# EdoardoBotta/RQ-VAE-Recommender

Hardware: AMD Instinct MI355X
Metric: item-embeddings quantized/sec (RQ-VAE fwd+bwd) (higher is better)
Workload: dtype f32 (MLP GEMMs f16x2-emulated)

## Files before the change

include/rqhip.h:

```cpp
#ifndef RQHIP_H
#define RQHIP_H

#include <stddef.h>
#include <stdint.h>

#ifdef __cplusplus
extern "C" {
#endif

#define RQHIP_VERSION 462

#define RQHIP_OK 0
#define RQHIP_EARG (-1)
#define RQHIP_EUNSUPPORTED (-2)
#define RQHIP_EWORKSPACE (-3)

#define RQHIP_MODE_EVAL 0
#define RQHIP_MODE_STE 1
#define RQHIP_MODE_ROTATION 2
#define RQHIP_MODE_GUMBEL 3

typedef void *rqhip_stream_t;

int rqhip_version(void);
// ... 336 lines not shown
    float *loss_rows;
    void *workspace;
    size_t workspace_bytes;
    const unsigned *a_row_max;
    int a_row_parts;
    unsigned *c_row_max;
    unsigned *c_col_max;
} rqhip_gemm_args;
int rqhip_gemm_split_supported(int Nc, int R);
size_t rqhip_weight_image_bytes(int Nc, int R, int arith);
int rqhip_weight_images(const rqhip_image_job *jobs, int n_jobs, rqhip_stream_t stream);
int rqhip_maxima(const float *A, const float *Y, float *masked_out, int64_t M, int R, unsigned *row_max, unsigned *col_max,
                 rqhip_stream_t stream);
size_t rqhip_gemm_split_recon_workspace_bytes(int64_t M, int Nc);
int rqhip_gemm_split_ex(const rqhip_gemm_args *args, rqhip_stream_t stream);
size_t rqhip_weight_planes_bytes(int Nc, int R);
int rqhip_weight_planes(const float *w, int rows, int cols, int transpose, void *planes, size_t planes_bytes,
                        rqhip_stream_t stream);
int rqhip_gemm_split(const float *A, int64_t M, int R, const void *planes, int Nc, int relu, float *C,
                     rqhip_stream_t stream);
int rqhip_gemm_split_recon(const float *A, int64_t M, int R, const void *planes, int Nc, const float *X, float row_scale,
                           float *G, float *loss_rows, void *workspace, size_t workspace_bytes, rqhip_stream_t stream);
int rqhip_recon_rescale_rows(const float *g_out, int64_t B, int N, float row_scale, float *g_spec, rqhip_stream_t stream);
int rqhip_recon_rescale_rows_ex(const float *g_out, int64_t B, int N, float row_scale, float *g_spec, unsigned *row_max,
                                int row_parts, unsigned *col_max, rqhip_stream_t stream);

typedef struct {
    int64_t B;
    int D;
    int H;
// ... 63 lines not shown
```

rq-vae-recommender_amd/csrc/gemm_split.hip:

```cpp
#include "rqhip_common.h"

namespace rqhip {

typedef float gs_f32x16 __attribute__((ext_vector_type(16)));
typedef float gs_f32x4 __attribute__((ext_vector_type(4)));
typedef float gs_f32x2 __attribute__((ext_vector_type(2)));
typedef __bf16 gs_bf16x8 __attribute__((ext_vector_type(8)));
typedef __bf16 gs_bf16x2 __attribute__((ext_vector_type(2)));
typedef _Float16 gs_f16x8 __attribute__((ext_vector_type(8)));
typedef _Float16 gs_f16x2 __attribute__((ext_vector_type(2)));
typedef unsigned gs_u32x2 __attribute__((ext_vector_type(2)));
typedef unsigned gs_u32x4 __attribute__((ext_vector_type(4)));
typedef int gs_i32x4 __attribute__((ext_vector_type(4)));

constexpr int kGsUB = 2;
constexpr int kGsK = 16;
constexpr int kGsColmaxLds = 1024;
constexpr int kGsTailWords = kWeightImageTailWords;

__device__ __forceinline__ void gs_split2(float a, float b, unsigned &h, unsigned &m, unsigned &l) {
    const gs_bf16x2 hh = __builtin_convertvector(gs_f32x2{a, b}, gs_bf16x2);
    h = __builtin_bit_cast(unsigned, hh);
    const float ra = a - __builtin_bit_cast(float, h << 16), rb = b - __builtin_bit_cast(float, h & 0xffff0000u);
    const gs_bf16x2 mm = __builtin_convertvector(gs_f32x2{ra, rb}, gs_bf16x2);
// ... 179 lines not shown
    int R, Nc;
    int n_col_tiles;
    unsigned n_big, n_tiles;
    int rt_big;
    unsigned *counter;
    int n_queues;
    int rt_fastest;
    int static_tiles;
    const float *X;
    float *rowsum;
    float row_scale;
    const unsigned *a_max;
    int a_parts;
    const int *b_exp;
    unsigned *c_rowmax, *c_colmax;
};

#ifndef GS_PROBE
#define GS_PROBE 0
#endif
#ifndef GS_PROLOGUE_ORDER
#define GS_PROLOGUE_ORDER 1
#endif
#ifndef GS_FAST_EPILOGUE
#define GS_FAST_EPILOGUE 1
#endif
#ifndef GS_REGION_PAD
#define GS_REGION_PAD 32
#endif

__device__ __forceinline__ unsigned gs_row16_umax(unsigned v) {
// ... 689 lines not shown
        if (!(tile & kSmallBit)) {
            const int ct = p.rt_fastest ? (int)(tile / rt_big) : (int)(tile % nct), rt = p.rt_fastest ? (int)(tile % rt_big) : (int)(tile / nct);
            gs_tile2<EPI, kBigRows / 32, COLS>(p, sbuf, s_aexp, s_colmax, (long long)rt * kBigRows, ct * COLS);
        } else {
            const unsigned st = tile & ~kSmallBit;
            const int ct = p.rt_fastest ? (int)(st / rt_small) : (int)(st % nct), rt = p.rt_fastest ? (int)(st % rt_small) : (int)(st / nct);
            gs_tile2<EPI, kSmallRows / 32, COLS>(p, sbuf, s_aexp, s_colmax, (long long)p.rt_big * kBigRows + (long long)rt * kSmallRows, ct * COLS);
        }
    }
    if (lds_colmax) {
        for (int c = tid; c < p.Nc; c += kThreads)
            if (s_colmax[c]) atomicMax(p.c_colmax + c, s_colmax[c]);
    }
}

__global__ __launch_bounds__(256) void recon_rows_finish_kernel(const float *__restrict__ rowsum, int nct, long long M,
                                                                float *__restrict__ out) {
    const long long m = (long long)blockIdx.x * 256 + threadIdx.x;
    if (m >= M) return;
    float s = rowsum[m];
    for (int c = 1; c < nct; ++c) s = s + rowsum[(size_t)c * M + m];
    out[m] = s;
}

}

using namespace rqhip;

static int gs_cols(int Nc) { return Nc % 256 == 0 ? 256 : 128; }
static int gs_np(int arith) { return arith == RQHIP_SPLIT_F16X2 ? 2 : arith == RQHIP_SPLIT_BF16X3 ? 3 : 0; }
// ... 49 lines not shown
    if (M < 0 || R <= 0 || (R % 4) != 0 || R > 16384 || (M > 0 && !A) || (masked_out && !Y) || !al16(A) || !al16(Y) || !al16(masked_out)) {
        set_error("maxima: bad arguments (R = %d must be a multiple of 4, at most 16384; 16-byte aligned rows; masked_out needs Y)", R);
        return RQHIP_EARG;
    }
    if (M == 0 || (!row_max && !col_max && !masked_out)) return RQHIP_OK;
    long long blocks = (M + 3) / 4;
    const long long cap = (long long)cu_count() * 8;
    if (blocks > cap) blocks = cap;
    hipStream_t s = reinterpret_cast<hipStream_t>(stream);
    profile_begin(s, RQHIP_PROF_MAXIMA, 0.0, (double)M * R * 4 * ((Y ? 2 : 1) + (masked_out ? 1 : 0)));
    hipLaunchKernelGGL(maxima_kernel, dim3((unsigned)blocks), dim3(256), col_max ? (size_t)R * 4 : 0, s, A, Y, masked_out, (long long)M, R,
                       row_max, col_max);
    profile_end(s);
    RQ_CHECK_LAUNCH("maxima_kernel");
    return RQHIP_OK;
}

extern "C" size_t rqhip_gemm_split_recon_workspace_bytes(int64_t M, int Nc) {
    return (M > 0 && Nc > 0 && Nc % 256 == 0) ? (size_t)(Nc / 256) * (size_t)M * sizeof(float) : 0;
}

extern "C" int rqhip_gemm_split_ex(const rqhip_gemm_args *a, rqhip_stream_t stream) {
    if (!a) {
        set_error("gemm_split: null argument block");
        return RQHIP_EARG;
    }
    const int np = gs_np(a->arith), epi = a->epilogue;
    const int64_t M = a->M;
    const int R = a->R, Nc = a->Nc;
    if (!np || M < 0 || !a->image || (M > 0 && (!a->A || !a->C)) || !rqhip_gemm_split_supported(Nc, R) || epi < 0 || epi > 3) {
// ... 61 lines not shown
        rt_big = 0;
        tiny = a->tile_rows == -11;
        small_rows = tiny ? 32 : 64;
    }
    if (!tile2 && (a->tile_rows == 256 || a->tile_rows == 128)) rt_big = rt_all;
    if (!tile2 && (a->tile_rows == 64 || a->tile_rows == 32)) rt_big = 0;
    const long long rem_rows = M - rt_big * big_rows > 0 ? M - rt_big * big_rows : 0;
    const long long rt_small = (rem_rows + small_rows - 1) / small_rows;
    p.rt_big = (int)rt_big;
    p.n_big = (unsigned)(rt_big * p.n_col_tiles);
    p.n_tiles = p.n_big + (unsigned)(rt_small * p.n_col_tiles);
    size_t lds = (tile2 && !occ4) ? (size_t)2 * 4 * (128 * 4 + 32) * 4 : (size_t)2 * (np * 2 * (big_rows + cols) * 16);
    const size_t lds_epi = gs_epilogue_lds(waves, big_rows, wide ? 8 : cols / 64);
    if (lds < lds_epi) lds = lds_epi;
    const long long tiles = (long long)p.n_tiles;
    const int grid = (int)(tiles < slots ? tiles : slots);
    auto go = [&](auto kern) -> int {
        static LdsGrant grant;
        RQ_RETURN_IF_HIP(grant.ensure(reinterpret_cast<const void *>(kern), (int)lds));
        profile_begin(s, RQHIP_PROF_GEMM_SPLIT, 2.0 * (double)M * Nc * R, 4.0 * (double)M * (R + Nc * (epi >= 2 ? 2 : 1)));
        hipLaunchKernelGGL(kern, dim3(grid), dim3(64 * waves), lds, s, p);
        profile_end(s);
        RQ_CHECK_LAUNCH("gemm_split_kernel");
        return 0;
    };
    int rc;
    if (occ4) {
        rc = epi == 3 ? go(gemm_split_kernel<3, 256, 2, 8, 128>) : epi == 1 ? go(gemm_split_kernel<1, 256, 2, 8, 128>) : go(gemm_split_kernel<0, 256, 2, 8, 128>);
    } else if (wide) {
        rc = epi == 3 ? go(gemm_f16_kernel<3, 512>) : epi == 1 ? go(gemm_f16_kernel<1, 512>) : go(gemm_f16_kernel<0, 512>);
    } else if (tile2 && tiny) {
        rc = epi == 3 ? go(gemm_f16_kernel<3, 256, 1>) : epi == 2 ? go(gemm_f16_kernel<2, 256, 1>) : epi == 1 ? go(gemm_f16_kernel<1, 256, 1>)
                                                                                                          : go(gemm_f16_kernel<0, 256, 1>);
    } else if (tile2) {
        rc = epi == 3 ? go(gemm_f16_kernel<3>) : epi == 2 ? go(gemm_f16_kernel<2>) : epi == 1 ? go(gemm_f16_kernel<1>) : go(gemm_f16_kernel<0>);
    } else if (np == 2) {
        rc = epi == 3 ? go(gemm_split_kernel<3, 128, 2, 4>) : epi == 1 ? go(gemm_split_kernel<1, 128, 2, 4>) : go(gemm_split_kernel<0, 128, 2, 4>);
    } else {
        if (epi == 3) {
            set_error("gemm_split: the masked epilogue exists for RQHIP_SPLIT_F16X2 only");
            return RQHIP_EUNSUPPORTED;
        }
// ... 33 lines not shown
```

rq-vae-recommender_amd/modules/encoder.py:

```python
from typing import List

import torch
from torch import Tensor, nn

from modules.normalize import L2NormalizationLayer
from rqhip import linear as _lin
from rqhip import ops, torch_ops
from rqhip.linear import use_split_gemms


def _grad_sink(w: Tensor):
    from rqhip.dist import claim_grad_sink
    return claim_grad_sink(w)


def _adopt(gw: Tensor, sink) -> Tensor:
    return gw.view_as(gw) if sink is not None else gw


def _plain(layers) -> bool:
    return all((isinstance(l, nn.Linear) and l.bias is None) or isinstance(l, nn.ReLU) for l in layers)


class _LinearReLU(torch.autograd.Function):
# ... 4 lines not shown
        ctx.save_for_backward(x, w, y if zero_bias is not None else None)
        return y

    @staticmethod
    def backward(ctx, gy: Tensor):
        x, w, y = ctx.saved_tensors
        need_x, need_w = ctx.needs_input_grad[0], ctx.needs_input_grad[1]
        sink = _grad_sink(w) if need_w else None
        gx, gw = _lin.backward(gy, y, x, w, need_x, need_w, sink)
        return gx, (_adopt(gw, sink) if need_w else None), None


class _MLPStack(torch.autograd.Function):

    @staticmethod
    def forward(ctx, x: Tensor, target, relus, zero_bias, given, defer, *weights):
        from rqhip import _lib
        from rqhip import autograd as _ag
        assert _lin.dense_f32(x), "_MLPStack takes a contiguous, 16-byte aligned fp32 ROCm matrix (MLP._run re-homes what is not)"
        n, M, R = len(weights), x.shape[0], _lin.Route
        need_w = [bool(f) for f in ctx.needs_input_grad[6:]]
        need_in = [bool(ctx.needs_input_grad[0]) or any(need_w[:i]) for i in range(n)]
        stack_jobs = _lin.wgrad_jobs_ok(M, [tuple(w.shape) for i, w in enumerate(weights) if need_w[i]])
        plans = [_lin.plan_layer(M, w.shape[0], w.shape[1], relu=relus[i], operands_aligned=True, weight_ok=_lin.dense_f32(w),
                                 need_dgrad=need_in[i], need_wgrad=need_w[i], stack_jobs=stack_jobs) for i, w in enumerate(weights)]
        imgs = iter(_lin.images([(w, False) for w, p in zip(weights, plans) if p.fwd == R.SPLIT]
                                + [(w, True) for w, p in zip(weights, plans) if p.dgrad == R.SPLIT]))
        img_f = [next(imgs) if p.fwd == R.SPLIT else None for p in plans]
        img_t = [next(imgs) if p.dgrad == R.SPLIT else None for p in plans]
        emit = [p.fwd in (R.SPLIT, R.SEAM_OUT) and (plans[i + 1].wgrad_f16 if i + 1 < n else (target is not None and p.wgrad_f16))
                for i, p in enumerate(plans)]
        col_outs = _lin.col_slices([w.shape[0] if e else 0 for w, e in zip(weights, emit)], x.device)
        acts, scs = [x], [given if given is not None else _lin.Scales()]
        if _lin.f16() and (plans[0].fwd == R.SPLIT or plans[0].wgrad_f16):
            _lin.ensure_scales(x, scs[0], plans[0].fwd == R.SPLIT, plans[0].wgrad_f16)
        out = g_recon = g_scales = None
# ... 10 lines not shown
                y, ysc = _lin.chain_forward(a, w, relus[i], want_rows=want_rows, col_out=col_outs[i])
            elif p.fwd == R.SPLIT:
                y, _, ysc = _lin.gemm(a, img_f[i], w.shape[0], epilogue=_lib.EPI_RELU if relus[i] else _lib.EPI_STORE,
                                      a_scales=sc, want_rows=want_rows, col_out=col_outs[i])
            elif p.fwd == R.SMALL:
                y, ysc = _lin.small_forward(a, w, relus[i]), _lin.Scales()
            else:
                y, ysc = _lin.library_forward(a, w, relus[i], zero_bias(w.shape[0], a) if relus[i] else None), _lin.Scales()
            acts.append(y)
            scs.append(ysc)
            out = y
        ctx.has_target = target is not None
        ctx.save_for_backward(x, *weights, target if ctx.has_target else out)
        ctx.acts_mid, ctx.scs, ctx.relus = (acts[1:] if ctx.has_target else acts[1:-1]), scs, tuple(relus)
        ctx.plans, ctx.stack_jobs, ctx.img_t, ctx.need_in, ctx.need_w = plans, stack_jobs, img_t, need_in, need_w
        ctx.defer = bool(defer)
        ctx.g_recon, ctx.g_scales, ctx.consumed = g_recon, g_scales, False
        return out

    @staticmethod
    def backward(ctx, g_out: Tensor):
        from rqhip import _lib
        x, weights, tail = ctx.saved_tensors[0], ctx.saved_tensors[1:-1], ctx.saved_tensors[-1]
        n, R = len(weights), _lin.Route
        target = tail if ctx.has_target else None
        acts = [x] + list(ctx.acts_mid) + ([] if ctx.has_target else [tail])
        scs, relus, need_in, need_w, plans = ctx.scs, ctx.relus, ctx.need_in, ctx.need_w, ctx.plans
        g_out = g_out.contiguous()
        handed = _lin.take_grad_handoff(g_out) if target is None else None
        if g_out.data_ptr() % 16 != 0:
            g_out = g_out.clone()
        if handed is not None:
            g, gsc = g_out, handed
        elif target is None:
            g, gsc = g_out, _lin.Scales()
        elif not ctx.consumed:
            ctx.consumed = True
            gsc = ctx.g_scales
            g = ops.recon_rescale_rows(ctx.g_recon, g_out, ctx.row_scale, gsc.rows, gsc.cols)
        else:
            g = ops.recon_loss_backward(acts[-1].mm(weights[-1].t()), target, g_out, True, False)[0]
            gsc = _lin.Scales()
        emit = [i > 0 and p.dgrad in (R.SPLIT, R.SEAM_OUT) and plans[i - 1].wgrad_f16 for i, p in enumerate(plans)]
        col_outs = _lin.col_slices([w.shape[1] if e else 0 for w, e in zip(weights, emit)], g.device)
        premasked = (not relus[n - 1]) or handed is not None
        gws = [None] * n
        own = []
        for i in range(n - 1, -1, -1):
            w, a, p = weights[i], acts[i], plans[i]
            y = acts[i + 1] if (relus[i] and not premasked) else None
            mask_on_load = p.dgrad == R.SEAM_IN and y is not None
            g_unmasked = g
            if p.wgrad == R.JOBS and ctx.stack_jobs:
                if y is not None:
                    g, gsc = torch.ops.aten.threshold_backward(g, y, 0.0), _lin.Scales()
                own.append((i, _lin.WgradJob(w, g, a, None, None, _grad_sink(w))))
            elif p.wgrad == R.F16_SPLIT_BATCHED and y is None:
                gsc = _lin.ensure_scales(g, gsc, False, True)
                own.append((i, _lin.WgradJob(w, g, a, gsc.cols, _lin.ensure_scales(a, scs[i], False, True).cols, _grad_sink(w))))
            elif need_w[i]:
# ... 5 lines not shown
                g, gsc = torch.ops.aten.threshold_backward(g, y, 0.0), _lin.Scales()
            if not need_in[i]:
                g = None
                break
            lower_relu = i > 0 and relus[i - 1]
            lower_split = i > 0 and plans[i - 1].dgrad == R.SPLIT
            if p.dgrad in (R.SEAM_IN, R.SEAM_OUT):
                if p.dgrad == R.SEAM_IN:
                    src, msk = (g_unmasked, y) if (mask_on_load and (g is None or g is g_unmasked)) else (g, None)
                    g, gsc = _lin.chain_input_grad(src, w, g_mask=msk)
                    premasked = not lower_relu
                else:
                    g, gsc = _lin.chain_input_grad(g, w, out_mask=a if lower_relu else None, want_rows=lower_split, col_out=col_outs[i])
                    premasked = True
            elif p.dgrad == R.SPLIT:
                fuse = _lin.f16() and lower_relu
                g, _, gsc = _lin.gemm(g, ctx.img_t[i], w.shape[1], epilogue=_lib.EPI_MASK if fuse else _lib.EPI_STORE,
                                      aux=a if fuse else None, a_scales=gsc, want_rows=lower_split and (fuse or not lower_relu),
                                      col_out=col_outs[i] if (fuse or not lower_relu) else None)
                premasked = fuse or not lower_relu
            elif p.dgrad == R.SMALL:
                g, gsc = _lin.small_input_grad(g, w, a if lower_relu else None), _lin.Scales()
                premasked = True
            else:
                g, gsc = g.mm(w), _lin.Scales()
                premasked = not lower_relu
        waited = _lin.wgrad_queue.take() if g_out.is_cuda else []
        jobs = [j for _, j in own]
        if jobs and not waited and ctx.defer and _lin.wgrad_queue.may_park(jobs):
            _lin.wgrad_queue.park(jobs)
            dws = [j.sink for j in jobs]
        else:
            dws = _lin.launch_wgrads(jobs, waited)
        for (i, j), dw in zip(own, dws):
            gws[i] = _adopt(dw, j.sink)
        return (g if ctx.needs_input_grad[0] else None), None, None, None, None, None, *gws


class MLP(nn.Module):
    def __init__(self, input_dim: int, hidden_dims: List[int], out_dim: int, dropout: float = 0.0,
                 normalize: bool = False) -> None:
        super().__init__()
        self.input_dim, self.hidden_dims, self.out_dim, self.dropout = input_dim, hidden_dims, out_dim, dropout
        widths = [input_dim, *hidden_dims, out_dim]
        stack = nn.Sequential()
        last = len(widths) - 2
        for i in range(len(widths) - 1):
            stack.append(nn.Linear(widths[i], widths[i + 1], bias=False))
            if i == last:
                break
            stack.append(nn.ReLU())
# ... 14 lines not shown
        assert x.shape[-1] == self.input_dim, f"Invalid input dim: Expected {self.input_dim}, found {x.shape[-1]}"
        if not (x.is_cuda and x.dim() == 2 and x.dtype == torch.float32):
            return self.mlp(x)
        return self._run(x if x.is_contiguous() else x.contiguous(), list(self.mlp))

    def _run(self, x: Tensor, layers, target: Tensor = None) -> Tensor:
        if torch_ops.enabled():
            return self._run_layerwise(x, layers)
        weights, relus, i = [], [], 0
        while i < len(layers) and isinstance(layers[i], nn.Linear) and layers[i].bias is None:
            relu = i + 1 < len(layers) and isinstance(layers[i + 1], nn.ReLU)
            weights.append(layers[i].weight)
            relus.append(relu)
            i += 2 if relu else 1
        if weights:
            given = _lin.attached_scales(x)
            if not _lin.dense_f32(x):
                x = x.clone(memory_format=torch.contiguous_format)
            x = _MLPStack.apply(x, target, tuple(relus), self._zero_bias, given, getattr(self, "_defer_wgrads", False), *weights)
        return self._run_layerwise(x, layers[i:]) if i < len(layers) else x

    def _run_layerwise(self, x: Tensor, layers) -> Tensor:
        as_ops = torch_ops.enabled()
        i = 0
        while i < len(layers):
            layer = layers[i]
            if (isinstance(layer, nn.Linear) and layer.bias is None and i + 1 < len(layers)
                    and isinstance(layers[i + 1], nn.ReLU)):
                x = (torch.ops.rqhip.linear_relu(x, layer.weight) if as_ops
                     else _LinearReLU.apply(x, layer.weight, self._zero_bias(layer.out_features, x)))
                i += 2
            elif isinstance(layer, nn.Linear) and layer.bias is None:
                x = torch.ops.rqhip.linear_plain(x, layer.weight) if as_ops else _LinearReLU.apply(x, layer.weight, None)
                i += 1
# ... 46 lines not shown
```

rq-vae-recommender_amd/modules/rqvae.py:

```python
from functools import cached_property
from typing import List, NamedTuple

import torch
from huggingface_hub import PyTorchModelHubMixin
from torch import Tensor, nn

from data.schemas import SeqBatch
from modules.encoder import MLP
from modules.loss import CategoricalReconstuctionLoss, ReconstructionLoss
from modules.normalize import l2norm
from modules.quantize import Quantize, QuantizeForwardMode
from rqhip import ops, torch_ops
from rqhip import linear as _lin
from rqhip.autograd import LossMeansFunction, RqSeamFunction, RqStackFunction

torch.set_float32_matmul_precision("highest")


FUSE_SEAM = True


_SIDE_STREAMS = {}


# ... 161 lines not shown
        n = self.n_cat_feats
        seam = self._seam_weights(xin)
        _lin.wgrad_queue.clear()
        reconstruction = x_hat = p_unique_ids = side = None
        if seam is not None:
            hidden = self.encoder.run_before_tail(xin)
            codebooks = torch.stack([layer.codebook() for layer in self.layers])
            sink = getattr(self, "_rq_cb_grad_sink", None)
            want_scales = _lin.f16() and xin.shape[0] >= _lin.SPLIT_MIN_ROWS
            if reducer is not None and hidden.requires_grad:
                hidden.register_hook(reducer.boundary_hook)
            ids, qloss, norms, d, d_rows, d_cols = RqSeamFunction.apply(hidden, seam[0], codebooks, seam[1], self.layers[0].hip_mode(),
                                                                        float(self.commitment_weight), sink, want_scales)
            if want_scales:
                _lin.attach_scales(d, d_rows, d_cols)
            st = _StackResult(None, None, ids, qloss, None, norms)
            if _lin.trims_on() and not torch.cuda.is_current_stream_capturing():
                side = _side_stream(ids.device)
                side.wait_stream(torch.cuda.current_stream())
                with torch.cuda.stream(side), torch.no_grad():
                    p_unique_ids = ops.unique_fraction(ids)
                ids.record_stream(side)
            if n == 0 and type(self.reconstruction_loss) is ReconstructionLoss and x.dim() == 2:
                reconstruction = self.decoder.reconstruction_rows(d, xin, first=2)
            if reconstruction is None:
                x_hat = self.decoder.run_after_head(d)
        else:
            res0 = self.encode(xin)
            if reducer is not None and res0.requires_grad:
                res0.register_hook(reducer.boundary_hook)
# ... 38 lines not shown
```

rq-vae-recommender_amd/rqhip/_lib.py:

```python
from __future__ import annotations

import ctypes as C
import os
import subprocess

import torch

_CSRC = os.path.join(os.path.dirname(os.path.dirname(os.path.abspath(__file__))), "csrc")
SO_PATH = os.path.join(_CSRC, "librqhip.so")

MODE_EVAL, MODE_STE, MODE_ROTATION, MODE_GUMBEL = 0, 1, 2, 3
FWD_SCAN_FP32, FWD_SCAN_VALU, FWD_NO_COOP_TAIL = 0x1, 0x2, 0x10
WGRAD_FP32 = 0x1
BWD_CBGRAD_MATRIX = 0x1
SPLIT_F16X2, SPLIT_BF16X3 = 0, 1
EPI_STORE, EPI_RELU, EPI_RECON, EPI_MASK = 0, 1, 2, 3
EARG = -1
ADAMW_TAIL_SCALARS = 8
PROF_TAGS = {1: "rq_forward", 2: "rq_backward", 3: "gemm_split", 4: "wgrad", 5: "maxima", 6: "weight_images", 7: "rq_seam", 8: "linear_small"}


class ImageJob(C.Structure):
    _fields_ = [("w", C.c_void_p), ("rows", C.c_int), ("cols", C.c_int), ("transpose", C.c_int), ("arith", C.c_int),
                ("image", C.c_void_p), ("image_bytes", C.c_size_t)]
# ... 162 lines not shown
    "rqhip_linear_wgrad_plan": (_int, [_i64, _int, _int, C.POINTER(_int)]),
    "rqhip_linear_wgrad_workspace_bytes": (_sz, [_i64, _int, _int]),
    "rqhip_linear_wgrad": (_int, [_vp, _vp, _vp, _i64, _int, _int, _vp, _vp, _vp, _sz, _vp]),
    "rqhip_linear_wgrad_ex": (_int, [_vp, _vp, _vp, _i64, _int, _int, _vp, _vp, _vp, _sz, C.c_uint, _vp]),
    "rqhip_linear_wgrad_f16": (_int, [_vp, _vp, _vp, _i64, _int, _int, _vp, _vp, _vp, _vp, _vp, _sz, _vp]),
    "rqhip_linear_wgrad_f16_batch_plan": (_int, [_i64, C.POINTER(_int), C.POINTER(_int), _int]),
    "rqhip_linear_wgrad_f16_batch_workspace_bytes": (_sz, [_i64, C.POINTER(_int), C.POINTER(_int), _int]),
    "rqhip_linear_wgrad_f16_batch": (_int, [C.POINTER(WgradJob), _int, _i64, _vp, _sz, _vp]),
    "rqhip_linear_wgrad_jobs_supported": (_int, [_int, _int]),
    "rqhip_linear_wgrad_jobs": (_int, [_vp, _vp, _vp, C.POINTER(_int), C.POINTER(_int), _int, _i64, _vp]),
    "rqhip_gemm_split_supported": (_int, [_int, _int]),
    "rqhip_weight_image_bytes": (_sz, [_int, _int, _int]),
    "rqhip_weight_images": (_int, [C.POINTER(ImageJob), _int, _vp]),
    "rqhip_maxima": (_int, [_vp, _vp, _vp, _i64, _int, _vp, _vp, _vp]),
    "rqhip_gemm_split_ex": (_int, [C.POINTER(GemmArgs), _vp]),
    "rqhip_weight_planes_bytes": (_sz, [_int, _int]),
    "rqhip_weight_planes": (_int, [_vp, _int, _int, _int, _vp, _sz, _vp]),
    "rqhip_gemm_split": (_int, [_vp, _i64, _int, _vp, _int, _int, _vp, _vp]),
    "rqhip_gemm_split_recon_workspace_bytes": (_sz, [_i64, _int]),
    "rqhip_gemm_split_recon": (_int, [_vp, _i64, _int, _vp, _int, _vp, _f32, _vp, _vp, _vp, _sz, _vp]),
    "rqhip_recon_rescale_rows": (_int, [_vp, _i64, _int, _f32, _vp, _vp]),
    "rqhip_recon_rescale_rows_ex": (_int, [_vp, _i64, _int, _f32, _vp, _vp, _int, _vp, _vp]),
    "rqhip_rq_seam_supported": (_int, [_int, _int, _int, _int]),
    "rqhip_rq_seam": (_int, [C.POINTER(SeamArgs), _vp]),
    "rqhip_linear_small_supported": (_int, [_i64, _int, _int]),
    "rqhip_linear_small_plan": (_int, [_i64, _int, _int, C.POINTER(_int), C.POINTER(_int)]),
    "rqhip_linear_small": (_int, [_vp, _vp, _int, _vp, _i64, _int, _int, _int, _vp, _int, _int, _vp]),
    "rqhip_adamw_step": (_int, [_vp, _vp, _vp, _vp, _vp, _int, _vp, _vp, _f32, _f32, _f32, _f32, _f32, _vp]),
    "rqhip_adamw_tail_workspace_bytes": (_i64, [_vp, _int]),
    "rqhip_adamw_tail_step": (_int, [_vp, _vp, _vp, _vp, _vp, _int, _vp, _vp, _vp, _vp, _sz, _f32, _f32, C.c_double, _i64, _f32, _f32,
# ... 47 lines not shown
```

rq-vae-recommender_amd/rqhip/autograd.py:

```python
from __future__ import annotations

from typing import Optional

import torch
from torch import Tensor

from . import ops


def _dense(g: Optional[Tensor]) -> Optional[Tensor]:
    if g is None:
        return None
    return g.contiguous()


class RqStackFunction(torch.autograd.Function):

    @staticmethod
    def forward(ctx, res0: Tensor, codebooks: Tensor, mode: int, beta: float, want_levels: bool, grad_sink=None):
        out = ops.rq_forward(res0, codebooks, mode, beta, want_embs=want_levels, want_residuals=want_levels)
        ctx.set_materialize_grads(False)
        ctx.save_for_backward(res0, codebooks, out.ids)
        ctx.mode, ctx.beta, ctx.want_levels, ctx.grad_sink = mode, beta, want_levels, grad_sink
        embs = out.embs if want_levels else res0.new_empty((0,))
# ... 46 lines not shown
        return r.ids, r.loss, r.embs_norm, r.out, rmax, cmax

    @staticmethod
    def backward(ctx, _g_ids, g_loss, _g_norm, g_d, _g_rmax=None, _g_cmax=None):
        from . import linear as _lin
        from .dist import claim_grad_sink
        h, w_in, codebooks, w_out, res0, ids, emb_sum, d = ctx.saved_tensors
        need_h, need_win, need_cb, need_wout = ctx.needs_input_grad[:4]
        g_d, g_loss = _dense(g_d), _dense(g_loss)
        B = h.shape[0]
        jobs = _lin.wgrad_jobs_ok(B, [tuple(w_out.shape), tuple(w_in.shape)])
        pending = []
        gw_out = gw_in = None
        g_es = None
        if g_d is not None:
            g_dm = None
            if need_wout:
                if jobs:
                    g_dm = torch.ops.aten.threshold_backward(g_d, d, 0.0)
                    pending.append(_lin.WgradJob(w_out, g_dm, emb_sum, None, None, claim_grad_sink(w_out)))
                else:
                    sink = claim_grad_sink(w_out)
                    gw, gp, _ = _lin.weight_grad(g_d, d, emb_sum, w_out, out=sink, want_masked=False)
                    gw_out = gw.view_as(gw) if sink is not None else gw
                    g_dm = gp if (gp is not None and gp is not g_d) else None
            if need_h or need_win or need_cb:
                g_es = (_lin.chain_input_grad(g_dm, w_out)[0] if g_dm is not None
                        else _lin.chain_input_grad(g_d, w_out, g_mask=d)[0])
        g_res0 = g_cb = None
        if need_h or need_win or need_cb:
            sink = ctx.grad_sink
            out_cb = None
            if need_cb and sink is not None and tuple(sink.view.shape) == tuple(codebooks.shape) and all(
                    p.grad is None and getattr(p, "_rq_sink_epoch", -1) != sink.owner.epoch for p in sink.params):
                out_cb = sink.view
                for p in sink.params:
                    p._rq_sink_epoch = sink.owner.epoch
            g_res0, g_cb = ops.rq_backward(res0, codebooks, ctx.mode, ctx.beta, ids, g_embsum=g_es, g_loss=g_loss,
                                           need_res0=need_h or need_win, need_codebooks=need_cb, out_g_codebooks=out_cb,
                                           cbgrad=ops.cbgrad_default())
# ... 329 lines not shown
```

rq-vae-recommender_amd/rqhip/linear.py:

```python
from enum import IntEnum
from typing import List, NamedTuple, Optional, Sequence, Tuple

import torch
from torch import Tensor

from . import _lib, ops

SPLIT_MIN_ROWS = 4096
_SPLIT_GEMMS = True
_ARITH = ops.F16X2
_FP32 = -1
_ARITH_NAMES = {"f16x2": ops.F16X2, "bf16x3": ops.BF16X3, "fp32": _FP32}


def use_split_gemms(on: bool = True) -> bool:
    global _SPLIT_GEMMS
    before, _SPLIT_GEMMS = _SPLIT_GEMMS, bool(on)
    return before


def use_arith(name: str) -> str:
    global _ARITH
    before = arith_name()
    _ARITH = _ARITH_NAMES[name]
# ... 66 lines not shown
    return [arena[sum(widths[:i]):sum(widths[:i + 1])] if n else None for i, n in enumerate(widths)]


_GRAD_HANDOFF: List[Optional[tuple]] = [None]


def handoff_grad(g: Tensor, sc: Scales) -> None:
    _GRAD_HANDOFF[0] = (g.data_ptr(), tuple(g.shape), g._version, sc)


def take_grad_handoff(g: Tensor) -> Optional[Scales]:
    slot, _GRAD_HANDOFF[0] = _GRAD_HANDOFF[0], None
    if slot is not None and slot[:3] == (g.data_ptr(), tuple(g.shape), g._version):
        return slot[3]
    return None


def ensure_scales(a: Tensor, sc: Optional[Scales], rows: bool, cols: bool) -> Scales:
    sc = sc if sc is not None else Scales()
    need_r, need_c = rows and sc.rows is None, cols and sc.cols is None
    if need_r or need_c:
        r, c, _ = ops.maxima(a, rows=need_r, cols=need_c)
        if need_r:
            sc.rows = r
        if need_c:
            sc.cols = c
    return sc


def _wide(n_cols: int) -> bool:
# ... 137 lines not shown
_STATIC_TILES = True


def use_static_tiles(on: bool = True) -> bool:
    global _STATIC_TILES
    before, _STATIC_TILES = _STATIC_TILES, bool(on)
    return before


def use_tiny_tiles(on: bool = True) -> bool:
    global _TINY_TILES
    before, _TINY_TILES = _TINY_TILES, bool(on)
    return before


def _tile_code(n_cols: int, n_red: int, epilogue: int) -> int:
    if _WIDE_TILES and f16() and n_cols % 512 == 0 and n_red >= _WIDE_MIN_RED and epilogue != _lib.EPI_RECON:
        return -5
    if not _STATIC_TILES:
        return -12
    return -9 if _TINY_TILES else 0


_CHAIN = True
CHAIN_D, CHAIN_H = 32, ops.SEAM_H


def use_chain_gemms(on: bool = True) -> bool:
    global _CHAIN
    before, _CHAIN = _CHAIN, bool(on)
    return before


def chain_gemms_on() -> bool:
    return _CHAIN
# ... 192 lines not shown
```

rq-vae-recommender_amd/rqhip/ops.py:

```python
from __future__ import annotations

import ctypes as C
from typing import NamedTuple, Optional

import torch
from torch import Tensor

from . import _lib
from ._lib import MODE_EVAL, MODE_GUMBEL, MODE_ROTATION, MODE_STE, RqHipError, check


def _need_gpu(*tensors: Optional[Tensor]) -> torch.device:
    dev = None
    for t in tensors:
        if t is None:
            continue
        if not t.is_cuda:
            raise RqHipError(
                "rqhip ops need ROCm device tensors (got a %s tensor); the HIP kernels are the only "
                "implementation of this path -- there is no CPU fallback." % t.device.type)
        if dev is None:
            dev = t.device
        elif t.device != dev:
            raise RqHipError(f"tensors on different devices: {dev} vs {t.device}")
# ... 1953 lines not shown
        rows = ws = None
        if epilogue == _lib.EPI_RECON:
            rows = torch.empty((M,), dtype=torch.float32, device=a.device)
            nbytes = l.rqhip_gemm_split_recon_workspace_bytes(M, int(n_cols))
            ws = torch.empty((max(nbytes, 4),), dtype=torch.uint8, device=a.device)
            args.loss_rows, args.workspace, args.workspace_bytes = rows.data_ptr(), ws.data_ptr(), nbytes
        if a_row_max is not None:
            args.a_row_max, args.a_row_parts = a_row_max.data_ptr(), a_row_max.shape[0]
        crm = torch.empty((n_cols // (256 if n_cols % 256 == 0 else 128), M), dtype=torch.int32, device=a.device) if want_row_max else None
        args.c_row_max, args.c_col_max = _ptr(crm), _ptr(col_max_out)
        import ctypes as C
        check(l.rqhip_gemm_split_ex(C.byref(args), _stream()), "rqhip_gemm_split_ex")
    return c, rows, crm


def gemm_split(a: Tensor, planes: Tensor, n_cols: int, relu: bool = False, tile_rows: int = 0, arith: int = BF16X3) -> Tensor:
    rm = maxima(a, cols=False)[0] if arith == F16X2 else None
    return gemm_split_ex(a, planes, n_cols, arith=arith, epilogue=_lib.EPI_RELU if relu else _lib.EPI_STORE, a_row_max=rm,
                         tile_rows=tile_rows)[0]


def gemm_split_recon(a: Tensor, planes: Tensor, n_cols: int, x: Tensor, row_scale: float, arith: int = BF16X3):
    if tuple(x.shape) != (a.shape[0], n_cols):
        raise RqHipError(f"gemm_split_recon: x is {tuple(x.shape)}, expected {(a.shape[0], n_cols)}")
    rm = maxima(a, cols=False)[0] if arith == F16X2 else None
    g, rows, _ = gemm_split_ex(a, planes, n_cols, arith=arith, epilogue=_lib.EPI_RECON, aux=x, row_scale=row_scale, a_row_max=rm)
    return g, rows


def recon_rescale_rows(g_spec: Tensor, g_out: Tensor, row_scale: float, row_max: Optional[Tensor] = None,
# ... 10 lines not shown
```

Measured before the change: 40.94 million.

## Add phase-staggered static GEMM tile schedule and fuse seam ReLU mask into dgrad

Adds new phase kernels for the f16x2 split GEMM that assign each block a contiguous range of row blocks. The first tile height is staggered by block class so that co-resident blocks fall out of lockstep, and tile sizes then shrink to cover the remainder. This is enabled by default for reductions of at most 512. Separately, the MLP backward now applies the ReLU mask of the quantizer output inside the first-layer dgrad epilogue and hands the masked gradient over, so the autograd path can skip a separate threshold_backward. Together these aim to cut tail and lockstep stalls on small-K GEMMs and to remove one elementwise pass, at the cost of more kernel variants and a more complex gradient handoff.

```diff
diff --git a/include/rqhip.h b/include/rqhip.h
--- a/include/rqhip.h
+++ b/include/rqhip.h
@@ -374,6 +374,7 @@
                  rqhip_stream_t stream);
 size_t rqhip_gemm_split_recon_workspace_bytes(int64_t M, int Nc);
 int rqhip_gemm_split_ex(const rqhip_gemm_args *args, rqhip_stream_t stream);
+int64_t rqhip_gemm_phase_plan(int64_t M, int Nc, int slots, int mode, int64_t *tiles, int64_t cap);
 size_t rqhip_weight_planes_bytes(int Nc, int R);
 int rqhip_weight_planes(const float *w, int rows, int cols, int transpose, void *planes, size_t planes_bytes,
                         rqhip_stream_t stream);
diff --git a/rq-vae-recommender_amd/csrc/gemm_split.hip b/rq-vae-recommender_amd/csrc/gemm_split.hip
--- a/rq-vae-recommender_amd/csrc/gemm_split.hip
+++ b/rq-vae-recommender_amd/csrc/gemm_split.hip
@@ -217,7 +217,41 @@
     int a_parts;
     const int *b_exp;
     unsigned *c_rowmax, *c_colmax;
+    unsigned ph_units, ph_q, ph_rem;
+    int ph_mode;
 };
+
+struct GsPhaseUnit {
+    unsigned blk0, nblk, open;
+};
+__host__ __device__ inline unsigned gs_phase_tile(unsigned left, unsigned max_ta) {
+    unsigned t = max_ta;
+    while (t > left) t >>= 1;
+    return t;
+}
+__host__ __device__ inline GsPhaseUnit gs_phase_unit(unsigned u, unsigned units, unsigned q, unsigned rem, unsigned max_ta, int mode) {
+    GsPhaseUnit r;
+    const unsigned first_long = units - rem;
+    r.blk0 = u * q + (u > first_long ? u - first_long : 0u);
+    r.nblk = q + (u >= first_long ? 1u : 0u);
+    const unsigned cls = (u / 8u) % 4u;
+    unsigned heights = 1u;
+    for (unsigned t = max_ta; t > 1u; t >>= 1) ++heights;
+    r.open = gs_phase_tile(r.nblk, max_ta);
+    if (mode == 2) {
+        const unsigned c = cls % heights;
+        if (c != 0u && (1u << (c - 1u)) < r.nblk) r.open = 1u << (c - 1u);
+    } else {
+        const unsigned parts = (r.nblk >= max_ta ? max_ta : 0u) | (r.nblk & (max_ta - 1u));
+        unsigned k = cls % (unsigned)__builtin_popcount(parts);
+        for (unsigned t = max_ta; t >= 1u; t >>= 1) {
+            if (!(parts & t)) continue;
+            if (k == 0u) { r.open = t; break; }
+            --k;
+        }
+    }
+    return r;
+}
 
 #ifndef GS_PROBE
 #define GS_PROBE 0
@@ -937,6 +971,63 @@
     }
 }
 
+template <int EPI>
+__global__ __launch_bounds__(256, 2) void gemm_f16_phase_kernel(const GemmSplitParams p) {
+    constexpr int kThreads = 256;
+    extern __shared__ __attribute__((aligned(16))) char gs_smem[];
+    unsigned *sbuf = reinterpret_cast<unsigned *>(gs_smem);
+    __shared__ int s_aexp[128];
+    __shared__ unsigned s_colmax[kGsColmaxLds];
+    const int tid = threadIdx.x;
+    const bool lds_colmax = p.c_colmax != nullptr && p.Nc <= kGsColmaxLds;
+    if (lds_colmax)
+        for (int c = tid; c < p.Nc; c += kThreads) s_colmax[c] = 0u;
+    const unsigned nct = (unsigned)p.n_col_tiles;
+    const GsPhaseUnit pu = gs_phase_unit(blockIdx.x / nct, p.ph_units, p.ph_q, p.ph_rem, 4u, p.ph_mode);
+    const int n0 = (int)(blockIdx.x % nct) * 256;
+    long long m0 = (long long)pu.blk0 * 32;
+    for (unsigned left = pu.nblk, ta = pu.open; left > 0u; left -= ta, ta = left ? gs_phase_tile(left, 4u) : 0u) {
+        __syncthreads();
+        if (ta == 4u) gs_tile2<EPI, 4, 256>(p, sbuf, s_aexp, s_colmax, m0, n0);
+        else if (ta == 2u) gs_tile2<EPI, 2, 256>(p, sbuf, s_aexp, s_colmax, m0, n0);
+        else gs_tile2<EPI, 1, 256>(p, sbuf, s_aexp, s_colmax, m0, n0);
+        m0 += 32ll * ta;
+    }
+    if (lds_colmax) {
+        __syncthreads();
+        for (int c = tid; c < p.Nc; c += kThreads)
+            if (s_colmax[c]) atomicMax(p.c_colmax + c, s_colmax[c]);
+    }
+}
+
+template <int EPI>
+__global__ __launch_bounds__(256, 2) void gemm_split_phase_kernel(const GemmSplitParams p) {
+    constexpr int kThreads = 256;
+    extern __shared__ __attribute__((aligned(16))) char gs_smem[];
+    unsigned *sbuf = reinterpret_cast<unsigned *>(gs_smem);
+    __shared__ int s_aexp[128];
+    __shared__ unsigned s_colmax[kGsColmaxLds];
+    const int tid = threadIdx.x;
+    const bool lds_colmax = p.c_colmax != nullptr && p.Nc <= kGsColmaxLds;
+    if (lds_colmax)
+        for (int c = tid; c < p.Nc; c += kThreads) s_colmax[c] = 0u;
+    const unsigned nct = (unsigned)p.n_col_tiles;
+    const GsPhaseUnit pu = gs_phase_unit(blockIdx.x / nct, p.ph_units, p.ph_q, p.ph_rem, 2u, p.ph_mode);
+    const int n0 = (int)(blockIdx.x % nct) * 128;
+    long long m0 = (long long)pu.blk0 * 64;
+    for (unsigned left = pu.nblk, ta = pu.open; left > 0u; left -= ta, ta = left ? gs_phase_tile(left, 2u) : 0u) {
+        __syncthreads();
+        if (ta == 2u) gs_tile<EPI, 2, 128, 2, 4>(p, sbuf, s_aexp, s_colmax, m0, n0);
+        else gs_tile<EPI, 1, 128, 2, 4>(p, sbuf, s_aexp, s_colmax, m0, n0);
+        m0 += 64ll * ta;
+    }
+    if (lds_colmax) {
+        __syncthreads();
+        for (int c = tid; c < p.Nc; c += kThreads)
+            if (s_colmax[c]) atomicMax(p.c_colmax + c, s_colmax[c]);
+    }
+}
+
 __global__ __launch_bounds__(256) void recon_rows_finish_kernel(const float *__restrict__ rowsum, int nct, long long M,
                                                                 float *__restrict__ out) {
     const long long m = (long long)blockIdx.x * 256 + threadIdx.x;
@@ -1016,6 +1107,53 @@
     profile_end(s);
     RQ_CHECK_LAUNCH("maxima_kernel");
     return RQHIP_OK;
+}
+
+struct GsPhaseHost {
+    int block_rows, cols;
+    unsigned max_ta, units, q, rem;
+};
+static bool gs_phase_host(int64_t M, int Nc, long long slots, GsPhaseHost &h) {
+    if (M <= 0 || Nc <= 0 || Nc % 128 != 0) return false;
+    h.cols = gs_cols(Nc);
+    h.block_rows = h.cols == 256 ? 32 : 64;
+    h.max_ta = 128 / h.block_rows;
+    const long long nct = Nc / h.cols, blocks = (M + h.block_rows - 1) / h.block_rows, cap = slots / nct;
+    if (cap < 1 || blocks > 0x7fffffffll) return false;
+    const long long units = blocks < cap ? blocks : cap;
+    h.units = (unsigned)units;
+    h.q = (unsigned)(blocks / units);
+    h.rem = (unsigned)(blocks % units);
+    return true;
+}
+
+extern "C" int64_t rqhip_gemm_phase_plan(int64_t M, int Nc, int slots, int mode, int64_t *tiles, int64_t cap) {
+    GsPhaseHost h;
+    if ((mode != 1 && mode != 2) || cap < 0 || (cap > 0 && !tiles) || !gs_phase_host(M, Nc, slots, h)) {
+        set_error("gemm_phase_plan: bad arguments (M = %lld > 0, Nc = %d a multiple of 128, slots = %d >= Nc's column tiles, mode 1 or 2)",
+                  (long long)M, Nc, slots);
+        return -1;
+    }
+    const int nct = Nc / h.cols;
+    int64_t n = 0;
+    for (unsigned u = 0; u < h.units; ++u) {
+        const GsPhaseUnit pu = gs_phase_unit(u, h.units, h.q, h.rem, h.max_ta, mode);
+        for (int ct = 0; ct < nct; ++ct) {
+            int64_t m0 = (int64_t)pu.blk0 * h.block_rows;
+            for (unsigned left = pu.nblk, ta = pu.open; left > 0u; left -= ta, ta = left ? gs_phase_tile(left, h.max_ta) : 0u) {
+                if (n < cap) {
+                    int64_t *t = tiles + 4 * n;
+                    t[0] = (int64_t)u * nct + ct;
+                    t[1] = m0;
+                    t[2] = (m0 + (int64_t)ta * h.block_rows <= M ? m0 + (int64_t)ta * h.block_rows : M) - m0;
+                    t[3] = (int64_t)ct * h.cols;
+                }
+                ++n;
+                m0 += (int64_t)ta * h.block_rows;
+            }
+        }
+    }
+    return n;
 }
 
 extern "C" size_t rqhip_gemm_split_recon_workspace_bytes(int64_t M, int Nc) {
@@ -1107,7 +1245,16 @@
     const size_t lds_epi = gs_epilogue_lds(waves, big_rows, wide ? 8 : cols / 64);
     if (lds < lds_epi) lds = lds_epi;
     const long long tiles = (long long)p.n_tiles;
-    const int grid = (int)(tiles < slots ? tiles : slots);
+    int grid = (int)(tiles < slots ? tiles : slots);
+    GsPhaseHost ph;
+    const bool phase = (a->tile_rows == -13 || a->tile_rows == -14) && np == 2 && gs_phase_host(M, Nc, slots, ph);
+    p.ph_units = p.ph_q = p.ph_rem = 0u;
+    p.ph_mode = 0;
+    if (phase) {
+        p.ph_units = ph.units; p.ph_q = ph.q; p.ph_rem = ph.rem;
+        p.ph_mode = a->tile_rows == -14 ? 2 : 1;
+        grid = (int)ph.units * p.n_col_tiles;
+    }
     auto go = [&](auto kern) -> int {
         static LdsGrant grant;
         RQ_RETURN_IF_HIP(grant.ensure(reinterpret_cast<const void *>(kern), (int)lds));
@@ -1118,7 +1265,12 @@
         return 0;
     };
     int rc;
-    if (occ4) {
+    if (phase && tile2) {
+        rc = epi == 3 ? go(gemm_f16_phase_kernel<3>) : epi == 2 ? go(gemm_f16_phase_kernel<2>) : epi == 1 ? go(gemm_f16_phase_kernel<1>)
+                                                                                                          : go(gemm_f16_phase_kernel<0>);
+    } else if (phase) {
+        rc = epi == 3 ? go(gemm_split_phase_kernel<3>) : epi == 1 ? go(gemm_split_phase_kernel<1>) : go(gemm_split_phase_kernel<0>);
+    } else if (occ4) {
         rc = epi == 3 ? go(gemm_split_kernel<3, 256, 2, 8, 128>) : epi == 1 ? go(gemm_split_kernel<1, 256, 2, 8, 128>) : go(gemm_split_kernel<0, 256, 2, 8, 128>);
     } else if (wide) {
         rc = epi == 3 ? go(gemm_f16_kernel<3, 512>) : epi == 1 ? go(gemm_f16_kernel<1, 512>) : go(gemm_f16_kernel<0, 512>);
diff --git a/rq-vae-recommender_amd/modules/encoder.py b/rq-vae-recommender_amd/modules/encoder.py
--- a/rq-vae-recommender_amd/modules/encoder.py
+++ b/rq-vae-recommender_amd/modules/encoder.py
@@ -42,12 +42,12 @@
 class _MLPStack(torch.autograd.Function):
 
     @staticmethod
-    def forward(ctx, x: Tensor, target, relus, zero_bias, given, defer, *weights):
+    def forward(ctx, x: Tensor, target, relus, zero_bias, given, defer, in_relu, *weights):
         from rqhip import _lib
         from rqhip import autograd as _ag
         assert _lin.dense_f32(x), "_MLPStack takes a contiguous, 16-byte aligned fp32 ROCm matrix (MLP._run re-homes what is not)"
         n, M, R = len(weights), x.shape[0], _lin.Route
-        need_w = [bool(f) for f in ctx.needs_input_grad[6:]]
+        need_w = [bool(f) for f in ctx.needs_input_grad[7:]]
         need_in = [bool(ctx.needs_input_grad[0]) or any(need_w[:i]) for i in range(n)]
         stack_jobs = _lin.wgrad_jobs_ok(M, [tuple(w.shape) for i, w in enumerate(weights) if need_w[i]])
         plans = [_lin.plan_layer(M, w.shape[0], w.shape[1], relu=relus[i], operands_aligned=True, weight_ok=_lin.dense_f32(w),
@@ -88,7 +88,7 @@
         ctx.save_for_backward(x, *weights, target if ctx.has_target else out)
         ctx.acts_mid, ctx.scs, ctx.relus = (acts[1:] if ctx.has_target else acts[1:-1]), scs, tuple(relus)
         ctx.plans, ctx.stack_jobs, ctx.img_t, ctx.need_in, ctx.need_w = plans, stack_jobs, img_t, need_in, need_w
-        ctx.defer = bool(defer)
+        ctx.defer, ctx.in_relu = bool(defer), bool(in_relu)
         ctx.g_recon, ctx.g_scales, ctx.consumed = g_recon, g_scales, False
         return out
 
@@ -118,6 +118,7 @@
         emit = [i > 0 and p.dgrad in (R.SPLIT, R.SEAM_OUT) and plans[i - 1].wgrad_f16 for i, p in enumerate(plans)]
         col_outs = _lin.col_slices([w.shape[1] if e else 0 for w, e in zip(weights, emit)], g.device)
         premasked = (not relus[n - 1]) or handed is not None
+        masked_for_producer = False
         gws = [None] * n
         own = []
         for i in range(n - 1, -1, -1):
@@ -153,7 +154,8 @@
                     g, gsc = _lin.chain_input_grad(g, w, out_mask=a if lower_relu else None, want_rows=lower_split, col_out=col_outs[i])
                     premasked = True
             elif p.dgrad == R.SPLIT:
-                fuse = _lin.f16() and lower_relu
+                fuse = _lin.f16() and (lower_relu or (i == 0 and ctx.in_relu))
+                masked_for_producer = i == 0 and fuse
                 g, _, gsc = _lin.gemm(g, ctx.img_t[i], w.shape[1], epilogue=_lib.EPI_MASK if fuse else _lib.EPI_STORE,
                                       aux=a if fuse else None, a_scales=gsc, want_rows=lower_split and (fuse or not lower_relu),
                                       col_out=col_outs[i] if (fuse or not lower_relu) else None)
@@ -164,6 +166,8 @@
             else:
                 g, gsc = g.mm(w), _lin.Scales()
                 premasked = not lower_relu
+        if masked_for_producer and g is not None and ctx.needs_input_grad[0]:
+            _lin.handoff_grad(g, _lin.Scales())
         waited = _lin.wgrad_queue.take() if g_out.is_cuda else []
         jobs = [j for _, j in own]
         if jobs and not waited and ctx.defer and _lin.wgrad_queue.may_park(jobs):
@@ -173,7 +177,7 @@
             dws = _lin.launch_wgrads(jobs, waited)
         for (i, j), dw in zip(own, dws):
             gws[i] = _adopt(dw, j.sink)
-        return (g if ctx.needs_input_grad[0] else None), None, None, None, None, None, *gws
+        return (g if ctx.needs_input_grad[0] else None), None, None, None, None, None, None, *gws
 
 
 class MLP(nn.Module):
@@ -218,10 +222,10 @@
             relus.append(relu)
             i += 2 if relu else 1
         if weights:
-            given = _lin.attached_scales(x)
+            given, in_relu = _lin.attached_scales(x), _lin.relu_output_marked(x)
             if not _lin.dense_f32(x):
                 x = x.clone(memory_format=torch.contiguous_format)
-            x = _MLPStack.apply(x, target, tuple(relus), self._zero_bias, given, getattr(self, "_defer_wgrads", False), *weights)
+            x = _MLPStack.apply(x, target, tuple(relus), self._zero_bias, given, getattr(self, "_defer_wgrads", False), in_relu, *weights)
         return self._run_layerwise(x, layers[i:]) if i < len(layers) else x
 
     def _run_layerwise(self, x: Tensor, layers) -> Tensor:
diff --git a/rq-vae-recommender_amd/modules/rqvae.py b/rq-vae-recommender_amd/modules/rqvae.py
--- a/rq-vae-recommender_amd/modules/rqvae.py
+++ b/rq-vae-recommender_amd/modules/rqvae.py
@@ -199,6 +199,7 @@
                                                                         float(self.commitment_weight), sink, want_scales)
             if want_scales:
                 _lin.attach_scales(d, d_rows, d_cols)
+            _lin.mark_relu_output(d)
             st = _StackResult(None, None, ids, qloss, None, norms)
             if _lin.trims_on() and not torch.cuda.is_current_stream_capturing():
                 side = _side_stream(ids.device)
diff --git a/rq-vae-recommender_amd/rqhip/_lib.py b/rq-vae-recommender_amd/rqhip/_lib.py
--- a/rq-vae-recommender_amd/rqhip/_lib.py
+++ b/rq-vae-recommender_amd/rqhip/_lib.py
@@ -200,6 +200,7 @@
     "rqhip_weight_images": (_int, [C.POINTER(ImageJob), _int, _vp]),
     "rqhip_maxima": (_int, [_vp, _vp, _vp, _i64, _int, _vp, _vp, _vp]),
     "rqhip_gemm_split_ex": (_int, [C.POINTER(GemmArgs), _vp]),
+    "rqhip_gemm_phase_plan": (_i64, [_i64, _int, _int, _int, C.POINTER(_i64), _i64]),
     "rqhip_weight_planes_bytes": (_sz, [_int, _int]),
     "rqhip_weight_planes": (_int, [_vp, _int, _int, _int, _vp, _sz, _vp]),
     "rqhip_gemm_split": (_int, [_vp, _i64, _int, _vp, _int, _int, _vp, _vp]),
diff --git a/rq-vae-recommender_amd/rqhip/autograd.py b/rq-vae-recommender_amd/rqhip/autograd.py
--- a/rq-vae-recommender_amd/rqhip/autograd.py
+++ b/rq-vae-recommender_amd/rqhip/autograd.py
@@ -84,16 +84,19 @@
         gw_out = gw_in = None
         g_es = None
         if g_d is not None:
-            g_dm = None
+            masked = _lin.take_grad_handoff(g_d) is not None
+            g_dm = g_d if masked else None
             if need_wout:
                 if jobs:
-                    g_dm = torch.ops.aten.threshold_backward(g_d, d, 0.0)
+                    if not masked:
+                        g_dm = torch.ops.aten.threshold_backward(g_d, d, 0.0)
                     pending.append(_lin.WgradJob(w_out, g_dm, emb_sum, None, None, claim_grad_sink(w_out)))
                 else:
                     sink = claim_grad_sink(w_out)
-                    gw, gp, _ = _lin.weight_grad(g_d, d, emb_sum, w_out, out=sink, want_masked=False)
+                    gw, gp, _ = _lin.weight_grad(g_d, d, emb_sum, w_out, out=sink, want_masked=False, premasked=masked)
                     gw_out = gw.view_as(gw) if sink is not None else gw
-                    g_dm = gp if (gp is not None and gp is not g_d) else None
+                    if not masked:
+                        g_dm = gp if (gp is not None and gp is not g_d) else None
             if need_h or need_win or need_cb:
                 g_es = (_lin.chain_input_grad(g_dm, w_out)[0] if g_dm is not None
                         else _lin.chain_input_grad(g_d, w_out, g_mask=d)[0])
diff --git a/rq-vae-recommender_amd/rqhip/linear.py b/rq-vae-recommender_amd/rqhip/linear.py
--- a/rq-vae-recommender_amd/rqhip/linear.py
+++ b/rq-vae-recommender_amd/rqhip/linear.py
@@ -104,6 +104,24 @@
     if slot is not None and slot[:3] == (g.data_ptr(), tuple(g.shape), g._version):
         return slot[3]
     return None
+
+
+_SEAM_MASK_ONCE = True
+
+
+def use_seam_mask_once(on: bool = True) -> bool:
+    global _SEAM_MASK_ONCE
+    before, _SEAM_MASK_ONCE = _SEAM_MASK_ONCE, bool(on)
+    return before
+
+
+def mark_relu_output(t: Tensor) -> Tensor:
+    t._rq_relu_out = True
+    return t
+
+
+def relu_output_marked(t: Tensor) -> bool:
+    return _SEAM_MASK_ONCE and bool(getattr(t, "_rq_relu_out", False))
 
 
 def ensure_scales(a: Tensor, sc: Optional[Scales], rows: bool, cols: bool) -> Scales:
@@ -271,11 +289,30 @@
     return before
 
 
+_PHASE_TILES = True
+_PHASE_MAX_RED = 512
+_PHASE_MODE = 0
+
+
+def use_phase_tiles(on: bool = True, max_red: Optional[int] = None, mode: Optional[int] = None) -> bool:
+    global _PHASE_TILES, _PHASE_MAX_RED, _PHASE_MODE
+    before, _PHASE_TILES = _PHASE_TILES, bool(on)
+    if max_red is not None:
+        _PHASE_MAX_RED = int(max_red)
+    if mode is not None:
+        assert mode in (0, 1, 2)
+        _PHASE_MODE = int(mode)
+    return before
+
+
 def _tile_code(n_cols: int, n_red: int, epilogue: int) -> int:
     if _WIDE_TILES and f16() and n_cols % 512 == 0 and n_red >= _WIDE_MIN_RED and epilogue != _lib.EPI_RECON:
         return -5
     if not _STATIC_TILES:
         return -12
+    if _PHASE_TILES and f16() and n_red <= _PHASE_MAX_RED:
+        mode = _PHASE_MODE or 1
+        return -13 if mode == 1 else -14
     return -9 if _TINY_TILES else 0
 
 
diff --git a/rq-vae-recommender_amd/rqhip/ops.py b/rq-vae-recommender_amd/rqhip/ops.py
--- a/rq-vae-recommender_amd/rqhip/ops.py
+++ b/rq-vae-recommender_amd/rqhip/ops.py
@@ -1991,6 +1991,17 @@
     return c, rows, crm
 
 
+def gemm_phase_plan(M: int, n_cols: int, slots: int, mode: int = 1):
+    import ctypes as C
+    l = _lib.lib()
+    n = l.rqhip_gemm_phase_plan(int(M), int(n_cols), int(slots), int(mode), None, 0)
+    if n < 0:
+        raise RqHipError(l.rqhip_last_error().decode())
+    buf = (C.c_int64 * (4 * max(n, 1)))()
+    assert l.rqhip_gemm_phase_plan(int(M), int(n_cols), int(slots), int(mode), buf, n) == n
+    return [tuple(buf[4 * i:4 * i + 4]) for i in range(n)]
+
+
 def gemm_split(a: Tensor, planes: Tensor, n_cols: int, relu: bool = False, tile_rows: int = 0, arith: int = BF16X3) -> Tensor:
     rm = maxima(a, cols=False)[0] if arith == F16X2 else None
     return gemm_split_ex(a, planes, n_cols, arith=arith, epilogue=_lib.EPI_RELU if relu else _lib.EPI_STORE, a_row_max=rm,
```

Result: no change. 41.04 million (median of 6 runs) (+0.3%).
